# Hamedkiri/heuristique_style_transfer_code

Hardware: NVIDIA B200
Metric: images/sec (higher is better)
Workload: dtype tf32

## Files before the change

heuristique_style_transfer_code_b200/_lib.py:

```python
from __future__ import annotations

import ctypes
import os
from ctypes import c_int, c_longlong, c_void_p, POINTER, c_uint

from .build import LIB_PATH

_LIB = None

GH_DTYPE_F32 = 0
GH_DTYPE_BF16 = 1
GH_ERR_BAD_ARG = -1
GH_ERR_UNSUPPORTED = -2

_P = c_void_p
_SIGNATURES = {
    "gh_version": (c_int, []),
    "gh_sm_count": (c_int, []),
    "gh_set_option": (c_int, [ctypes.c_char_p, c_int]),
    "gh_last_device_error": (c_int, [POINTER(c_uint)]),
    "gh_gram_pool_fwd": (c_int, [_P, c_int, c_longlong, c_longlong, c_longlong, c_int, c_int, c_int, c_int, _P, c_int,
                                  c_int, c_int, c_int, _P]),
    "gh_gram_dense_fwd": (c_int, [_P, c_int, c_longlong, c_longlong, c_longlong, c_int, c_int, c_int, _P, c_int, c_int,
                                   _P]),
    "gh_adaptive_pool_fwd": (c_int, [_P, c_int, c_int, c_int, _P, c_int, c_int, _P]),
    "gh_adaptive_pool_bwd": (c_int, [_P, c_int, c_int, c_int, c_int, c_int, _P, _P]),
    "gh_gram_pool_bwd": (c_int, [_P, c_int, c_longlong, c_longlong, c_longlong, c_int, c_int, c_int, c_int, _P, c_int,
                                  c_int, _P, c_int, c_longlong, c_longlong, c_longlong, c_int, _P]),
    "gh_gram_dense_bwd": (c_int, [_P, c_int, c_longlong, c_longlong, c_longlong, c_int, c_int, c_int, _P, _P, c_int,
                                   c_longlong, c_longlong, c_longlong, c_int, _P]),
    "gh_attn_head_fwd": (c_int, [_P] * 7 + [c_int] * 4 + [_P] * 5 + [_P]),
    "gh_transpose_cast": (c_int, [_P, c_int, _P, c_int, c_int, c_int, c_int, c_longlong, _P]),
    "gh_preprocess_frame": (c_int, [_P, c_longlong, c_int, c_int, c_int, _P, _P, _P, c_int, _P, _P, _P, c_int, _P, _P, _P,
                                     c_int, c_int, _P]),
    "gh_normalize_u8": (c_int, [_P, _P, c_longlong, c_int, c_longlong, _P, _P, _P]),
    "gh_gemm_f32": (c_int, [_P, c_longlong, c_longlong, _P, c_longlong, c_longlong, _P, _P, c_longlong, c_int, c_int,
                             c_int, _P]),
    "gh_maxpool2d_nhwc": (c_int, [_P, c_int, _P] + [c_int] * 7 + [_P]),
    "gh_stem_space_to_depth": (c_int, [_P] + [c_longlong] * 4 + [c_int] * 3 + [_P, c_int, _P]),
    "gh_stem_conv_pool_nhwc": (c_int, [_P] + [c_longlong] * 4 + [c_int] * 3 + [_P] * 4),
    "gh_stem_conv_pool_u8_nhwc": (c_int, [_P] + [c_longlong] * 4 + [c_int] * 3 + [_P] * 6),
    "gh_patch_gram_workspace": (c_longlong, [c_int, c_int, c_int]),
    "gh_patch_gram_fwd": (c_int, [_P, _P, _P, _P, c_int, c_int, c_int, c_int, _P, _P, _P, _P]),
    "gh_patch_attn_fwd": (c_int, [_P] * 11 + [c_int] * 5 + [_P, _P, _P]),
    "gh_attn_head_bwd_workspace": (c_longlong, [c_int, c_int, c_int]),
    "gh_attn_head_bwd": (c_int, [_P] * 10 + [c_int] * 4 + [_P] * 8 + [_P]),
    "gh_gram_mse_blocks": (c_int, [c_longlong]),
    "gh_gram_mse": (c_int, [_P, _P, c_longlong, _P, _P, _P]),
    "gh_split_bf16": (c_int, [_P, _P, c_longlong, c_longlong, _P]),
    "gh_gemm_planes": (c_int, [_P, c_longlong, c_longlong, c_int, _P, c_longlong, c_longlong, c_int, _P, _P, _P,
                                c_longlong, c_longlong, c_int, c_int, c_int, c_int, _P]),
    "gh_tgemm_plan": (c_int, [c_int, c_int, c_int, c_int, c_int, POINTER(c_int), POINTER(c_int), POINTER(c_int)]),
    "gh_gram_bwd_plan": (c_int, [c_int, c_int, c_int, c_int, c_int, POINTER(c_int)]),
    "gh_attn_head_fwd2": (c_int, [_P] * 7 + [c_int] * 4 + [_P] * 6 + [_P]),
    "gh_attn_head_bwd2_workspace": (c_longlong, [c_int, c_int, c_int]),
    "gh_attn_head_bwd2": (c_int, [_P] * 10 + [c_int] * 4 + [_P] * 8 + [_P]),
}
EXPORTED_SYMBOLS = tuple(_SIGNATURES)


class GramHeadError(RuntimeError):
    pass


def library_path() -> str:
    return os.environ.get("GRAMHEAD_LIB", LIB_PATH)


def lib() -> ctypes.CDLL:
    global _LIB
    if _LIB is None:
        path = library_path()
        if not os.path.isfile(path):
            raise GramHeadError(
                f"gramhead: {path} not found. Build it with `python -m heuristique_style_transfer_code_b200.build` "
                "(needs nvcc, targets sm_100a). There is no CPU or PyTorch fallback for the Gram + attention head.")
        handle = ctypes.CDLL(path)
        for name, (res, args) in _SIGNATURES.items():
            fn = getattr(handle, name)
            fn.restype = res
            fn.argtypes = args
        _LIB = handle
        _apply_env_options(handle)
    return _LIB


def _apply_env_options(handle) -> None:
    spec = os.environ.get("GRAMHEAD_OPTIONS", "").strip()
    if not spec:
        return
    for item in spec.split(","):
        name, sep, value = item.strip().partition("=")
        if not sep or not name:
            raise GramHeadError(f"gramhead: GRAMHEAD_OPTIONS: expected name=value, got {item!r}")
# ... 23 lines not shown
```

heuristique_style_transfer_code_b200/build.py:

```python
from __future__ import annotations

import os
import shutil
import subprocess

CSRC = os.path.join(os.path.dirname(os.path.abspath(__file__)), "csrc")
LIB_PATH = os.path.join(CSRC, "libgramhead.so")
SOURCES = ["gramhead.cu", "common.cuh", "gram_fwd.cuh", "pair.cuh", "gram_fwd_pair.cuh", "gram_bwd2.cuh", "gram_bwd_pair.cuh",
           "umma_gemm.cuh", "tgemm_pair.cuh", "launch.cuh", "attn_head.cuh", "attn_head2.cuh", "preprocess.cuh", "transpose.cuh", "patchgan.cuh", "pool.cuh", "stem.cuh", "style_loss.cuh"]
NVCC_FLAGS = ["-gencode", "arch=compute_100a,code=sm_100a", "-O3", "-lineinfo", "-std=c++17",
              "-Xcompiler", "-fPIC", "-shared"]


def _nvcc() -> str:
    for cand in (os.environ.get("NVCC"), shutil.which("nvcc"), "/usr/local/cuda/bin/nvcc"):
        if cand and os.path.isfile(cand):
            return cand
    raise RuntimeError("gramhead: nvcc not found (set NVCC=/path/to/nvcc)")


def is_stale() -> bool:
    if not os.path.isfile(LIB_PATH):
        return True
    built = os.path.getmtime(LIB_PATH)
    deps = [os.path.join(CSRC, s) for s in SOURCES]
    deps.append(os.path.join(os.path.dirname(os.path.dirname(CSRC)), "include", "gramhead.h"))
    return any(os.path.getmtime(d) > built for d in deps if os.path.isfile(d))


def build_library(force: bool = False, verbose: bool = False) -> str:
    if not force and not is_stale():
        return LIB_PATH
    cmd = [_nvcc(), *NVCC_FLAGS, "gramhead.cu", "-o", LIB_PATH + ".tmp"]
    if verbose:
        cmd.insert(1, "-Xptxas=-v")
    res = subprocess.run(cmd, cwd=CSRC, capture_output=True, text=True)
    if res.returncode != 0:
        raise RuntimeError("gramhead: nvcc failed\n" + res.stdout + res.stderr)
    if verbose:
        print(res.stderr)
    os.replace(LIB_PATH + ".tmp", LIB_PATH)
    return LIB_PATH


if __name__ == "__main__":
    print(build_library(force=True, verbose=True))
```

heuristique_style_transfer_code_b200/csrc/gramhead.cu:

```cuda
#include "../../include/gramhead.h"
#include "common.cuh"
#include "gram_fwd.cuh"
#include "gram_fwd_pair.cuh"
#include "gram_bwd2.cuh"
#include "gram_bwd_pair.cuh"
#include "attn_head.cuh"
#include "umma_gemm.cuh"
#include "tgemm_pair.cuh"
#include "attn_head2.cuh"
#include "preprocess.cuh"
#include "transpose.cuh"
#include "patchgan.cuh"
#include "pool.cuh"
#include "stem.cuh"
#include "style_loss.cuh"
#include <string>

namespace gh {

static int sm_count_cached() {
  static int cached[64] = {0};
  int dev = 0;
  if (cudaGetDevice(&dev) != cudaSuccess || dev < 0 || dev >= 64) return 148;
  if (cached[dev] == 0) {
    int n = 0;
    if (cudaDeviceGetAttribute(&n, cudaDevAttrMultiProcessorCount, dev) != cudaSuccess || n <= 0) n = 148;
    cached[dev] = n;
    error_record_host();
  }
  return cached[dev];
}

static int ilog2_exact(int v) {
  if (v <= 0 || (v & (v - 1))) return -1;
  int s = 0;
  while ((1 << s) < v) ++s;
  return s;
}

static int choose_ksplit(long long base_units, int nkb, int ctas, bool balance = false) {
  if (base_units >= ctas) {
    if (!balance) return 1;
    const long long r1 = (base_units + ctas - 1) / ctas * 2, r2 = (2 * base_units + ctas - 1) / ctas;
    return (nkb >= 8 && r2 * 100 <= r1 * 93) ? 2 : 1;
  }
  long long ks = (2LL * ctas + base_units - 1) / base_units;
  const int kmax = nkb / 2 > 1 ? nkb / 2 : 1;
  if (ks > kmax) ks = kmax;
  if (ks > 128) ks = 128;
  return ks < 1 ? 1 : (int)ks;
}

static cudaError_t gemm_auto(const float* A, long long a_sm, long long a_sk, const float* Bm, long long b_sk,
                             long long b_sn, const float* bias, float* D, long long ldd, int M, int N, int K,
                             int accumulate, cudaStream_t st) {
  if (!accumulate && (a_sk == 1 || a_sm == 1) && (b_sk == 1 || b_sn == 1)) {
    const bool a_mn = (a_sk != 1), b_mn = (b_sk != 1);
    cudaError_t e = launch_umma_gemm(A, a_mn, a_mn ? a_sk : a_sm, Bm, b_mn, b_mn ? b_sk : b_sn, bias, D, ldd, M, N, K,
                                     sm_count_cached(), st);
    if (e != cudaErrorNotSupported) return e;
  }
  return launch_sgemm(A, a_sm, a_sk, Bm, b_sk, b_sn, bias, D, ldd, M, N, K, accumulate, st);
}

template <int SRC, int KP>
static cudaError_t launch_gram_fwd_one(const GramFwdParams& p, int grid, cudaStream_t st) {
  cudaError_t e = cudaFuncSetAttribute(gram_fwd_kernel<SRC, KP>, cudaFuncAttributeMaxDynamicSharedMemorySize,
// ... 614 lines not shown
  if (p.OH <= 0 || p.OW <= 0) return GH_ERR_BAD_ARG;
  p.total_vec = (long long)B * p.OH * p.OW * (C / vec);
  const int cv = C / vec;
  if (cv > 256 || B > 65535) return GH_ERR_UNSUPPORTED;
  const int ppc = 256 / cv;
  const dim3 grid((p.OW + ppc - 1) / ppc, (p.OH + kPoolRows - 1) / kPoolRows, B);
  if (grid.y > 65535) return GH_ERR_UNSUPPORTED;
  if (dtype == GH_DTYPE_F32) maxpool2d_nhwc_kernel<float><<<grid, 256, 0, (cudaStream_t)stream>>>(p);
  else maxpool2d_nhwc_kernel<__nv_bfloat16><<<grid, 256, 0, (cudaStream_t)stream>>>(p);
  return (int)cudaGetLastError();
}

int gh_stem_space_to_depth(const float* x, long long img_stride, long long c_stride, long long y_stride,
                           long long x_stride, int B, int H, int W, void* z, int z_dtype, void* stream) {
  if (!x || !z || B <= 0 || H <= 0 || W <= 0) return GH_ERR_BAD_ARG;
  if (z_dtype != GH_DTYPE_F32 && z_dtype != GH_DTYPE_BF16) return GH_ERR_BAD_ARG;
  if ((H & 1) || (W & 1) || (uintptr_t)z % 16 != 0) return GH_ERR_UNSUPPORTED;
  StemS2DParams p{};
  p.x = x; p.z = z; p.s_img = img_stride; p.s_c = c_stride; p.s_y = y_stride; p.s_x = x_stride;
  p.B = B; p.H = H; p.W = W; p.HP = H / 2 + 3; p.WP = W / 2 + 3;
  p.total = (long long)B * p.HP * p.WP;
  const long long want = (p.total + 255) / 256;
  const long long cap = (long long)gh_sm_count() * 32;
  const int grid = (int)(want < cap ? want : cap);
  if (z_dtype == GH_DTYPE_F32) stem_space_to_depth_kernel<float><<<grid, 256, 0, (cudaStream_t)stream>>>(p);
  else stem_space_to_depth_kernel<__nv_bfloat16><<<grid, 256, 0, (cudaStream_t)stream>>>(p);
  return (int)cudaGetLastError();
}

int gh_stem_conv_pool_nhwc(const float* x, long long img_stride, long long c_stride, long long y_stride,
                           long long x_stride, int B, int H, int W, const float* w_packed, const float* bias, float* out,
                           void* stream) {
  if (!x || !w_packed || !bias || !out || B <= 0 || H <= 0 || W <= 0) return GH_ERR_BAD_ARG;
  if ((H & 1) || (W & 1) || (uintptr_t)w_packed % 16 != 0 || (uintptr_t)out % 16 != 0) return GH_ERR_UNSUPPORTED;
  StemConvPoolParams<float> p{};
  p.x = x; p.w = w_packed; p.bias = bias; p.out = out;
  return stem_conv_pool_launch(p, img_stride, c_stride, y_stride, x_stride, B, H, W, stream);
}

int gh_stem_conv_pool_u8_nhwc(const unsigned char* x, long long img_stride, long long c_stride, long long y_stride,
                              long long x_stride, int B, int H, int W, const float* mean3_host, const float* std3_host,
                              const float* w_packed, const float* bias, float* out, void* stream) {
  if (!x || !mean3_host || !std3_host || !w_packed || !bias || !out || B <= 0 || H <= 0 || W <= 0) return GH_ERR_BAD_ARG;
  StemConvPoolParams<uint8_t> p{};
  for (int c = 0; c < 3; ++c) {
    if (!(std3_host[c] != 0.f && std3_host[c] == std3_host[c])) return GH_ERR_BAD_ARG;
    p.mean[c] = mean3_host[c]; p.std[c] = std3_host[c];
  }
  if ((H & 1) || (W & 1) || (uintptr_t)w_packed % 16 != 0 || (uintptr_t)out % 16 != 0) return GH_ERR_UNSUPPORTED;
  p.x = x; p.w = w_packed; p.bias = bias; p.out = out;
  return stem_conv_pool_launch(p, img_stride, c_stride, y_stride, x_stride, B, H, W, stream);
}

int gh_gram_mse_blocks(long long n) {
  if (n <= 0) return 0;
  long long blocks = (n / 4 + kMseThreads - 1) / kMseThreads;
  const long long cap = (long long)sm_count_cached() * 4 < kMseMaxBlocks ? (long long)sm_count_cached() * 4 : kMseMaxBlocks;
  if (blocks > cap) blocks = cap;
  return (int)(blocks < 1 ? 1 : blocks);
}

int gh_gram_mse(const float* G, const float* G_target, long long n, float* dG, float* partial, void* stream) {
  if (!G || !G_target || !dG || !partial || n <= 0) return GH_ERR_BAD_ARG;
  if (n % 4 != 0 || ((uintptr_t)G | (uintptr_t)G_target | (uintptr_t)dG) % 16 != 0) return GH_ERR_UNSUPPORTED;
  gram_mse_kernel<<<gh_gram_mse_blocks(n), kMseThreads, 0, (cudaStream_t)stream>>>(G, G_target, dG, partial, n / 4,
                                                                                   1.0f / (float)n);
  return (int)cudaGetLastError();
}

long long gh_patch_gram_workspace(int L, int B, int D) {
  if (L <= 0 || B <= 0 || D <= 0) return 0;
  return (long long)L * B * D * (kPatchBins + 4);
}

int gh_patch_gram_fwd(const float* const* maps, const int* H, const int* W, const long long* strides, int L, int B,
                      int D, int ln_input, float* gram, float* gram_norm, float* workspace, void* stream) {
  if (!maps || !H || !W || !strides || !gram || !gram_norm || !workspace || L <= 0 || B <= 0 || D <= 0)
    return GH_ERR_BAD_ARG;
  if ((uintptr_t)workspace % 8 != 0) return GH_ERR_BAD_ARG;
  if (L > kPatchMaxLayers || D > kPatchMaxD || B > 0x7fffffff / 2) return GH_ERR_UNSUPPORTED;
  PatchGramParams p{};
  for (int l = 0; l < L; ++l) {
    if (!maps[l] || H[l] <= 0 || W[l] <= 0) return GH_ERR_BAD_ARG;
    p.layer[l].x = maps[l];
    p.layer[l].H = H[l];
    p.layer[l].W = W[l];
    p.layer[l].s_img = strides[4 * l + 0];
    p.layer[l].s_c = strides[4 * l + 1];
    p.layer[l].s_y = strides[4 * l + 2];
    p.layer[l].s_x = strides[4 * l + 3];
  }
  p.L = L; p.B = B; p.D = D; p.ln_input = ln_input ? 1 : 0;
  p.gram = gram; p.gram_norm = gram_norm;
  const long long planes = (long long)L * B * D;
  double* stats = reinterpret_cast<double*>(workspace);
  float* pooled = workspace + planes * 4;
  const long long gx = (long long)B * ((D + 7) / 8);
  if (gx > 0x7fffffffLL) return GH_ERR_UNSUPPORTED;
  patch_pool_kernel<<<dim3((unsigned)gx, L), kPatchThreads, (kPatchThreads / 32) * kPatchSmallPlane * sizeof(float),
                      (cudaStream_t)stream>>>(p, pooled, stats);
  cudaError_t e = cudaGetLastError();
  if (e != cudaSuccess) return (int)e;
  const size_t smem = (size_t)D * kPatchBins * 4 + 32 * sizeof(double);
  patch_gram_kernel<<<dim3(B, L), kPatchThreads, smem, (cudaStream_t)stream>>>(p, pooled, stats);
  return (int)cudaGetLastError();
}
// ... 240 lines not shown
```

heuristique_style_transfer_code_b200/frozen_encoder.py:

```python
from __future__ import annotations

import os
from typing import List, Optional, Tuple

import torch
import torch.nn as nn
import torch.nn.functional as F

from . import ops

STEM_SPACE_TO_DEPTH = os.environ.get("GRAMHEAD_STEM_S2D", "1") != "0"


def _stem_space_to_depth_weight(weight: torch.Tensor) -> torch.Tensor:
    o = weight.shape[0]
    w8 = weight.new_zeros((o, 3, 8, 8))
    w8[:, :, 1:, 1:] = weight
    w12 = w8.view(o, 3, 4, 2, 4, 2).permute(0, 1, 3, 5, 2, 4).reshape(o, 12, 4, 4)
    w16 = weight.new_zeros((o, 16, 4, 4))
    w16[:, :12] = w12
    return w16.contiguous(memory_format=torch.channels_last)


def _tf32_round(x: torch.Tensor) -> torch.Tensor:
    bits = (x.contiguous().view(torch.int32).to(torch.int64) & 0xFFFFFFFF) + 0x1000
    bits = bits & 0xFFFFE000
    return torch.where(bits >= 2 ** 31, bits - 2 ** 32, bits).to(torch.int32).view(torch.float32)


def pack_stem_weight(w16: torch.Tensor) -> torch.Tensor:
    w = _tf32_round(w16.float().contiguous())
    return w.view(64, 2, 2, 4, 4, 4).permute(4, 5, 1, 2, 0, 3).contiguous().view(-1)


def _fold(conv: nn.Conv2d, bn: nn.BatchNorm2d, dtype: torch.dtype, channels_last: bool):
    var, mean = bn.running_var.detach().float(), bn.running_mean.detach().float()
    gamma = bn.weight.detach().float() if bn.weight is not None else torch.ones_like(var)
    beta = bn.bias.detach().float() if bn.bias is not None else torch.zeros_like(var)
    scale = gamma * torch.rsqrt(var + bn.eps)
    weight = conv.weight.detach().float() * scale.view(-1, 1, 1, 1)
    bias = beta - mean * scale
    if conv.bias is not None:
        bias = bias + conv.bias.detach().float() * scale
    weight = weight.to(dtype).contiguous(memory_format=torch.channels_last if channels_last else torch.contiguous_format)
    return weight, bias.to(dtype).contiguous(), conv.stride, conv.padding, conv.dilation, conv.groups


def _foldable(conv, bn) -> bool:
    return (isinstance(conv, nn.Conv2d) and type(bn) is nn.BatchNorm2d and bn.track_running_stats
            and bn.running_mean is not None and bn.running_var is not None and conv.padding_mode == "zeros"
            and not isinstance(conv.padding, str))


def _is_bottleneck(block) -> bool:
    names = ("conv1", "bn1", "conv2", "bn2", "conv3", "bn3", "relu", "downsample")
    if type(block).__name__ != "Bottleneck" or not all(hasattr(block, n) for n in names):
        return False
    if not isinstance(block.relu, nn.ReLU):
        return False
    ok = _foldable(block.conv1, block.bn1) and _foldable(block.conv2, block.bn2) and _foldable(block.conv3, block.bn3)
    if block.downsample is not None:
        ds = block.downsample
        ok = ok and isinstance(ds, nn.Sequential) and len(ds) == 2 and _foldable(ds[0], ds[1])
    return ok


def encoder_signature(encoder: nn.Module) -> Optional[Tuple]:
    try:
        return tuple((t.data_ptr(), t._version) for t in list(encoder.parameters()) + list(encoder.buffers()))
    except RuntimeError:
        return None


class FoldedEncoder:

    def __init__(self, stem, pool, stages, signature, dtype, channels_last):
        self.stem, self.pool, self.stages = stem, pool, stages
        self.stem_s2d = None
        self.stem_packed = None
        self._stem_fused = True
        self.signature, self.dtype, self.channels_last = signature, dtype, channels_last

    @staticmethod
    def supported(encoder: nn.Sequential) -> bool:
        if len(encoder) < 4:
            return False
        if not (_foldable(encoder[0], encoder[1]) and isinstance(encoder[2], nn.ReLU) and isinstance(encoder[3], nn.MaxPool2d)):
            return False
        for stage in list(encoder)[4:]:
            if not isinstance(stage, nn.Sequential) or not all(_is_bottleneck(b) for b in stage):
                return False
        return True

    @classmethod
    def build(cls, encoder: nn.Sequential, dtype: torch.dtype, channels_last: bool) -> Optional["FoldedEncoder"]:
        if not cls.supported(encoder):
            return None
        with torch.no_grad():
            stem = _fold(encoder[0], encoder[1], dtype, channels_last)
            conv1 = encoder[0]
            stem_s2d = None
            if (STEM_SPACE_TO_DEPTH and channels_last and conv1.in_channels == 3 and conv1.kernel_size == (7, 7)
                    and conv1.stride == (2, 2) and conv1.padding == (3, 3) and conv1.dilation == (1, 1) and conv1.groups == 1):
                stem_s2d = (_stem_space_to_depth_weight(stem[0].float()).to(dtype), stem[1], (1, 1), (0, 0), (1, 1), 1)
            stages: List[list] = []
            for stage in list(encoder)[4:]:
                blocks = []
                for b in stage:
                    c3 = _fold(b.conv3, b.bn3, dtype, channels_last)
                    down = None
                    if b.downsample is not None:
                        dw, db, *geom = _fold(b.downsample[0], b.downsample[1], torch.float32, channels_last)
                        bias3 = (c3[1].float() + db).to(dtype)
                        c3 = (c3[0], bias3) + tuple(c3[2:])
                        down = (dw.to(dtype).contiguous(memory_format=torch.channels_last if channels_last
                                                        else torch.contiguous_format), None) + tuple(geom)
                    blocks.append((_fold(b.conv1, b.bn1, dtype, channels_last), _fold(b.conv2, b.bn2, dtype, channels_last),
                                   c3, down))
                stages.append(blocks)
        plan = cls(stem, encoder[3], stages, encoder_signature(encoder), dtype, channels_last)
        plan.stem_s2d = stem_s2d
        pool = encoder[3]
        if (stem_s2d is not None and dtype == torch.float32 and conv1.out_channels == 64
                and pool.kernel_size in (3, (3, 3)) and pool.stride in (2, (2, 2)) and pool.padding in (1, (1, 1))
                and pool.dilation in (1, (1, 1)) and not pool.ceil_mode and not pool.return_indices):
            plan.stem_packed = pack_stem_weight(stem_s2d[0])
        return plan

    @staticmethod
    def _conv_relu(x, p):
        w, b, stride, padding, dilation, groups = p
        return torch.cudnn_convolution_relu(x, w, b, stride, padding, dilation, groups)

    def _pool(self, x):
        p = self.pool
        k, s, pad = p.kernel_size, p.stride, p.padding
        plain = (isinstance(k, int) and isinstance(s, int) and isinstance(pad, int) and p.dilation == 1
                 and not p.ceil_mode and not p.return_indices)
        vec = 4 if x.dtype == torch.float32 else 8
        if plain and self.channels_last and x.shape[1] % vec == 0 and x.is_contiguous(memory_format=torch.channels_last):
            return ops.maxpool2d_nhwc(x, k, s, pad)
        return p(x)

    def _fused_stem_applies(self, x: torch.Tensor) -> bool:
        return (self.stem_packed is not None and self._stem_fused and torch.backends.cudnn.allow_tf32
                and x.dim() == 4 and x.shape[1] == 3 and x.shape[2] % 2 == 0 and x.shape[3] % 2 == 0)

    def stem_forward(self, x: torch.Tensor, normalize=None) -> torch.Tensor:
        if normalize is not None and x.dtype == torch.uint8:
            if self._fused_stem_applies(x):
                return ops.stem_conv_pool_u8(x, *normalize, self.stem_packed, self.stem_s2d[1])
            x = ops.normalize_u8(x, *normalize)
        if x.dtype == torch.float32 and self._fused_stem_applies(x):
            return ops.stem_conv_pool(x, self.stem_packed, self.stem_s2d[1])
        if (self.stem_s2d is not None and x.dtype == torch.float32 and x.shape[1] == 3 and x.shape[2] % 2 == 0
                and x.shape[3] % 2 == 0):
            x = self._conv_relu(ops.stem_space_to_depth(x, self.dtype), self.stem_s2d)
        else:
            x = x.to(self.dtype)
            if self.channels_last:
                x = x.contiguous(memory_format=torch.channels_last)
            x = self._conv_relu(x, self.stem)
        return self._pool(x)

    def __call__(self, x: torch.Tensor, normalize=None):
        x = self.stem_forward(x, normalize)
        outs = []
        for blocks in self.stages:
            for c1, c2, c3, down in blocks:
                identity = x
                y = self._conv_relu(x, c1)
                y = self._conv_relu(y, c2)
                if down is not None:
                    identity = F.conv2d(x, down[0], down[1], down[2], down[3], down[4], down[5])
                w, b, stride, padding, dilation, groups = c3
                x = torch.cudnn_convolution_add_relu(y, w, identity, 1.0, b, stride, padding, dilation, groups)
            outs.append(x)
        return x, outs
```

heuristique_style_transfer_code_b200/ops.py:

```python
from __future__ import annotations

import ctypes
from typing import List, Optional, Sequence, Tuple

import torch

from . import _lib
from ._lib import GH_DTYPE_BF16, GH_DTYPE_F32, GramHeadError, check

KSPLIT = 0
MAX_CTAS = 0

LAUNCHES = 0
PROFILE = None


class _Timed:
    def __init__(self, name, kernels, device, **work):
        self.name, self.kernels, self.device, self.work = name, kernels, device, work

    def __enter__(self):
        global LAUNCHES
        LAUNCHES += self.kernels
        if PROFILE is not None:
# ... 201 lines not shown
    with torch.cuda.device(a.device), _Timed(f"gemm_f32[M={m},N={n},K={k}]", 1, a.device, **work):
        rc = _lib.lib().gh_gemm_f32(a.data_ptr(), a.stride(0), a.stride(1), b.data_ptr(), b.stride(0), b.stride(1),
                                    0 if bias is None else bias.data_ptr(), out.data_ptr(), n, m, n, k, _stream_ptr(a))
    check(rc, "gh_gemm_f32")
    return out


def maxpool2d_nhwc(x: torch.Tensor, kernel: int, stride: int, padding: int) -> torch.Tensor:
    _require_cuda(x, "x")
    if x.dim() != 4 or not x.is_contiguous(memory_format=torch.channels_last):
        raise GramHeadError("gramhead: maxpool2d_nhwc takes a channels_last (B, C, H, W) tensor")
    b, c, h, w = x.shape
    oh, ow = (h + 2 * padding - kernel) // stride + 1, (w + 2 * padding - kernel) // stride + 1
    out = torch.empty((b, c, oh, ow), device=x.device, dtype=x.dtype, memory_format=torch.channels_last)
    work = dict(bytes=(x.numel() + out.numel()) * x.element_size(), flops=0, kind="maxpool")
    with torch.cuda.device(x.device), _Timed(f"maxpool2d_nhwc[C={c},HW={h}x{w},{x.dtype}]", 1, x.device, **work):
        rc = _lib.lib().gh_maxpool2d_nhwc(x.data_ptr(), _dtype_code(x), out.data_ptr(), b, h, w, c, kernel, stride, padding,
                                          _stream_ptr(x))
    check(rc, "gh_maxpool2d_nhwc")
    return out


def stem_space_to_depth(x: torch.Tensor, dtype: torch.dtype) -> torch.Tensor:
    _require_cuda(x, "x")
    if x.dim() != 4 or x.shape[1] != 3 or x.dtype != torch.float32 or x.shape[2] % 2 or x.shape[3] % 2:
        raise GramHeadError("gramhead: stem_space_to_depth takes fp32 (B, 3, H, W) images with even H and W")
    b, _, h, w = x.shape
    z = torch.empty((b, 16, h // 2 + 3, w // 2 + 3), device=x.device, dtype=dtype, memory_format=torch.channels_last)
    work = dict(bytes=x.numel() * 4 + z.numel() * z.element_size(), flops=0, kind="stem_s2d")
    with torch.cuda.device(x.device), _Timed(f"stem_space_to_depth[HW={h}x{w},{dtype}]", 1, x.device, **work):
        rc = _lib.lib().gh_stem_space_to_depth(x.data_ptr(), x.stride(0), x.stride(1), x.stride(2), x.stride(3), b, h, w,
                                               z.data_ptr(), _dtype_code(z), _stream_ptr(x))
    check(rc, "gh_stem_space_to_depth")
    return z


def stem_conv_pool(x: torch.Tensor, packed_weight: torch.Tensor, bias: torch.Tensor) -> torch.Tensor:
    _require_cuda(x, "x")
    if x.dim() != 4 or x.shape[1] != 3 or x.dtype != torch.float32 or x.shape[2] % 2 or x.shape[3] % 2:
        raise GramHeadError("gramhead: stem_conv_pool takes fp32 (B, 3, H, W) images with even H and W")
    if (packed_weight.dtype != torch.float32 or packed_weight.numel() != 16384 or not packed_weight.is_contiguous()
            or bias.dtype != torch.float32 or bias.numel() != 64 or not bias.is_contiguous()
            or packed_weight.device != x.device or bias.device != x.device):
        raise GramHeadError("gramhead: stem_conv_pool takes the packed fp32 stem weights (16384) and bias (64) on x's device")
    b, _, h, w = x.shape
    oh, ow = h // 2, w // 2
    ph, pw = (oh - 1) // 2 + 1, (ow - 1) // 2 + 1
    out = torch.empty((b, 64, ph, pw), device=x.device, dtype=torch.float32, memory_format=torch.channels_last)
    work = dict(bytes=(x.numel() + out.numel()) * 4, flops=2 * b * oh * ow * 64 * 147, kind="stem_conv_pool")
    with torch.cuda.device(x.device), _Timed(f"stem_conv_pool[HW={h}x{w}]", 1, x.device, **work):
        rc = _lib.lib().gh_stem_conv_pool_nhwc(x.data_ptr(), x.stride(0), x.stride(1), x.stride(2), x.stride(3), b, h, w,
                                               packed_weight.data_ptr(), bias.data_ptr(), out.data_ptr(), _stream_ptr(x))
    check(rc, "gh_stem_conv_pool_nhwc")
    return out


def stem_conv_pool_u8(x: torch.Tensor, mean, std, packed_weight: torch.Tensor, bias: torch.Tensor) -> torch.Tensor:
    _require_cuda(x, "x")
    if x.dim() != 4 or x.shape[1] != 3 or x.dtype != torch.uint8 or x.shape[2] % 2 or x.shape[3] % 2:
        raise GramHeadError("gramhead: stem_conv_pool_u8 takes uint8 (B, 3, H, W) images with even H and W")
    if (packed_weight.dtype != torch.float32 or packed_weight.numel() != 16384 or not packed_weight.is_contiguous()
            or bias.dtype != torch.float32 or bias.numel() != 64 or not bias.is_contiguous()
            or packed_weight.device != x.device or bias.device != x.device):
        raise GramHeadError("gramhead: stem_conv_pool_u8 takes the packed fp32 stem weights (16384) and bias (64) on x's device")
    mean, std = [float(v) for v in mean], [float(v) for v in std]
    if len(mean) != 3 or len(std) != 3:
        raise GramHeadError("gramhead: stem_conv_pool_u8: 3 channels need 3 means and stds")
    b, _, h, w = x.shape
    oh, ow = h // 2, w // 2
    ph, pw = (oh - 1) // 2 + 1, (ow - 1) // 2 + 1
    out = torch.empty((b, 64, ph, pw), device=x.device, dtype=torch.float32, memory_format=torch.channels_last)
    fl = ctypes.c_float * 3
    work = dict(bytes=x.numel() + out.numel() * 4, flops=2 * b * oh * ow * 64 * 147, kind="stem_conv_pool")
    with torch.cuda.device(x.device), _Timed(f"stem_conv_pool_u8[HW={h}x{w}]", 1, x.device, **work):
        rc = _lib.lib().gh_stem_conv_pool_u8_nhwc(x.data_ptr(), x.stride(0), x.stride(1), x.stride(2), x.stride(3), b, h,
                                                  w, fl(*mean), fl(*std), packed_weight.data_ptr(), bias.data_ptr(),
                                                  out.data_ptr(), _stream_ptr(x))
    check(rc, "gh_stem_conv_pool_u8_nhwc")
    return out


def normalize_u8_host(t: torch.Tensor, mean, std) -> torch.Tensor:
    shape = (1, -1, 1, 1)
    out = t.to(torch.float32).div_(255)
    return out.sub_(torch.tensor(mean, dtype=torch.float32).view(shape)).div_(torch.tensor(std, dtype=torch.float32).view(shape))


def normalize_u8(x: torch.Tensor, mean, std, out: Optional[torch.Tensor] = None) -> torch.Tensor:
    _require_cuda(x, "x")
    if x.dim() != 4 or x.dtype != torch.uint8 or not 1 <= x.shape[1] <= 4:
        raise GramHeadError("gramhead: normalize_u8 takes a (B, C <= 4, H, W) uint8 batch")
    mean, std = [float(v) for v in mean], [float(v) for v in std]
    b, c, h, w = x.shape
    if len(mean) != c or len(std) != c:
        raise GramHeadError(f"gramhead: normalize_u8: {c} channels need {c} means and stds")
    x = x.contiguous()
    if out is None:
        out = torch.empty((b, c, h, w), device=x.device, dtype=torch.float32)
    else:
        if (out.dtype != torch.float32 or out.device != x.device or out.dim() != 4 or out.shape[0] < b
                or out.shape[1:] != x.shape[1:] or not out.is_contiguous()):
            raise GramHeadError("gramhead: normalize_u8: `out` must be a dense fp32 (>= B, C, H, W) tensor on x's device")
        out = out[:b]
    if b == 0:
        return out
    fl = ctypes.c_float * c
# ... 349 lines not shown
```

include/gramhead.h:

```cpp
#ifndef GRAMHEAD_H_
#define GRAMHEAD_H_

#ifdef __cplusplus
extern "C" {
#endif

#define GH_ERR_BAD_ARG (-1)
#define GH_ERR_UNSUPPORTED (-2)

#define GH_DTYPE_F32 0
#define GH_DTYPE_BF16 1

int gh_version(void);

int gh_sm_count(void);

int gh_set_option(const char* name, int value);

int gh_last_device_error(unsigned int* out4);

int gh_gram_pool_fwd(const void* F, int f_dtype, long long img_stride, long long row_stride, long long x_stride, int B,
                     int C, int HW, int g, float* desc, int l, int L, int ksplit, int max_ctas, void* stream);

int gh_gram_dense_fwd(const void* F, int f_dtype, long long img_stride, long long row_stride, long long x_stride, int B,
                      int C, int HW, float* G, int ksplit, int max_ctas, void* stream);

int gh_adaptive_pool_fwd(const float* G, int B, int C, int g, float* desc, int l, int L, void* stream);
int gh_adaptive_pool_bwd(const float* d_desc, int l, int L, int B, int C, int g, float* dG, void* stream);

int gh_gram_pool_bwd(const void* F, int f_dtype, long long img_stride, long long row_stride, long long x_stride, int B,
                     int C, int HW, int g, const float* d_desc, int l, int L, void* dF, int df_dtype,
                     long long df_img_stride, long long df_row_stride, long long df_x_stride, int max_ctas, void* stream);

int gh_gram_dense_bwd(const void* F, int f_dtype, long long img_stride, long long row_stride, long long x_stride, int B,
                      int C, int HW, const float* dG, void* dF, int df_dtype, long long df_img_stride,
                      long long df_row_stride, long long df_x_stride, int max_ctas, void* stream);

int gh_attn_head_fwd(const float* desc, const float* W_in, const float* b_in, const float* W_out, const float* b_out,
                     const float* W_c, const float* b_c, int B, int L, int E, int nc, float* qkv, float* probs,
                     float* obar, float* emb, float* logits, void* stream);

int gh_transpose_cast(const void* in, int in_dtype, void* out, int out_dtype, int B, int R, int S, long long out_pitch,
                      void* stream);

int gh_preprocess_frame(const unsigned char* frame, long long pitch_bytes, int H, int W, int bgr, const int* hx_min,
                        const int* hx_size, const int* hk, int hkmax, const int* vy_min, const int* vy_size, const int* vk,
                        int vkmax, const float* mean3_host, const float* std3_host, float* out, int OH, int OW,
                        void* stream);

int gh_normalize_u8(const unsigned char* src, float* dst, long long images, int channels, long long hw,
                    const float* mean_host, const float* std_host, void* stream);

int gh_gemm_f32(const float* A, long long a_sm, long long a_sk, const float* B, long long b_sk, long long b_sn,
                const float* bias, float* D, long long ldd, int M, int N, int K, void* stream);

int gh_maxpool2d_nhwc(const void* in, int dtype, void* out, int B, int H, int W, int C, int k, int stride, int pad,
                      void* stream);

int gh_stem_space_to_depth(const float* x, long long img_stride, long long c_stride, long long y_stride,
                           long long x_stride, int B, int H, int W, void* z, int z_dtype, void* stream);

int gh_stem_conv_pool_nhwc(const float* x, long long img_stride, long long c_stride, long long y_stride,
                           long long x_stride, int B, int H, int W, const float* w_packed, const float* bias, float* out,
                           void* stream);

int gh_stem_conv_pool_u8_nhwc(const unsigned char* x, long long img_stride, long long c_stride, long long y_stride,
                              long long x_stride, int B, int H, int W, const float* mean3_host, const float* std3_host,
                              const float* w_packed, const float* bias, float* out, void* stream);

long long gh_patch_gram_workspace(int L, int B, int D);
int gh_patch_gram_fwd(const float* const* maps, const int* H, const int* W, const long long* strides, int L, int B,
                      int D, int ln_input, float* gram, float* gram_norm, float* workspace, void* stream);

int gh_patch_attn_fwd(const float* feat, const float* W_in1, const float* b_in1, const float* W_out1,
                      const float* b_out1, const float* W_in2, const float* b_in2, const float* W_out2,
                      const float* b_out2, const float* W_c, const float* b_c, int L, int B, int E, int heads, int nc,
                      float* emb, float* logits, void* stream);

long long gh_attn_head_bwd_workspace(int B, int L, int E);

int gh_attn_head_bwd(const float* desc, const float* W_in, const float* W_out, const float* W_c, const float* qkv,
                     const float* probs, const float* obar, const float* emb, const float* d_logits,
                     const float* d_emb_ext, int B, int L, int E, int nc, float* d_desc, float* dW_in, float* db_in,
                     float* dW_out, float* db_out, float* dW_c, float* db_c, float* workspace, void* stream);

int gh_gram_mse_blocks(long long n);
int gh_gram_mse(const float* G, const float* G_target, long long n, float* dG, float* partial, void* stream);

int gh_split_bf16(const float* src, void* planes, long long n, long long plane_stride, void* stream);

int gh_gemm_planes(const void* A_planes, long long lda, long long a_plane_stride, int a_mn, const void* B_planes,
                   long long ldb, long long b_plane_stride, int b_mn, const float* bias, float* D, void* D_planes,
                   long long ldd, long long d_plane_stride, int M, int N, int K, int max_split, void* stream);

int gh_tgemm_plan(int M, int N, int K, int max_split, int npairs, int* tn, int* ksplit, int* units);

int gh_gram_bwd_plan(int C, int HW, int g, int f_dtype, int channels_last, int* out);

int gh_attn_head_fwd2(const float* desc, const void* w_in_planes, const float* b_in, const void* w_out_planes,
                      const float* b_out, const float* W_c, const float* b_c, int B, int L, int E, int nc, void* x_planes,
                      float* qkv, float* probs, void* obar_planes, float* emb, float* logits, void* stream);

long long gh_attn_head_bwd2_workspace(int B, int L, int E);

int gh_attn_head_bwd2(const void* x_planes, const void* w_in_planes, const void* w_out_planes, const float* W_c,
                      const float* qkv, const float* probs, const void* obar_planes, const float* emb,
                      const float* d_logits, const float* d_emb_ext, int B, int L, int E, int nc, float* d_desc,
                      float* dW_in, float* db_in, float* dW_out, float* db_out, float* dW_c, float* db_c, void* workspace,
                      void* stream);

#ifdef __cplusplus
}
#endif
#endif
```

Baseline: 46110.

## Fuse ResNet downsample shortcut and conv3 into one tcgen05 GEMM kernel

Adds a warp-specialized tcgen05 TF32 GEMM kernel that computes the first bottleneck block's 1x1 conv3 and 1x1 downsample shortcut as one K=128 GEMM over the concatenated inputs, then applies bias, the residual sum and ReLU from TMEM in a single pass. This replaces a separate downsample conv, an intermediate identity tensor and a cuDNN conv-add-relu call, cutting memory traffic and launches for that block. It applies only to fp32 channels_last blocks with 64->256 1x1 convs. Producer warps load and TF32-round the activations into shared memory, accumulators are double-buffered in TMEM, and the weights stay resident in shared memory. Summing the two bias vectors is assumed to happen when the packed bias is built.

```diff
diff --git a/heuristique_style_transfer_code_b200/_lib.py b/heuristique_style_transfer_code_b200/_lib.py
--- a/heuristique_style_transfer_code_b200/_lib.py
+++ b/heuristique_style_transfer_code_b200/_lib.py
@@ -40,6 +40,7 @@
     "gh_stem_space_to_depth": (c_int, [_P] + [c_longlong] * 4 + [c_int] * 3 + [_P, c_int, _P]),
     "gh_stem_conv_pool_nhwc": (c_int, [_P] + [c_longlong] * 4 + [c_int] * 3 + [_P] * 4),
     "gh_stem_conv_pool_u8_nhwc": (c_int, [_P] + [c_longlong] * 4 + [c_int] * 3 + [_P] * 6),
+    "gh_conv3_shortcut_relu_nhwc": (c_int, [_P, _P, c_longlong, _P, _P, _P, _P]),
     "gh_patch_gram_workspace": (c_longlong, [c_int, c_int, c_int]),
     "gh_patch_gram_fwd": (c_int, [_P, _P, _P, _P, c_int, c_int, c_int, c_int, _P, _P, _P, _P]),
     "gh_patch_attn_fwd": (c_int, [_P] * 11 + [c_int] * 5 + [_P, _P, _P]),
diff --git a/heuristique_style_transfer_code_b200/build.py b/heuristique_style_transfer_code_b200/build.py
--- a/heuristique_style_transfer_code_b200/build.py
+++ b/heuristique_style_transfer_code_b200/build.py
@@ -7,7 +7,8 @@
 CSRC = os.path.join(os.path.dirname(os.path.abspath(__file__)), "csrc")
 LIB_PATH = os.path.join(CSRC, "libgramhead.so")
 SOURCES = ["gramhead.cu", "common.cuh", "gram_fwd.cuh", "pair.cuh", "gram_fwd_pair.cuh", "gram_bwd2.cuh", "gram_bwd_pair.cuh",
-           "umma_gemm.cuh", "tgemm_pair.cuh", "launch.cuh", "attn_head.cuh", "attn_head2.cuh", "preprocess.cuh", "transpose.cuh", "patchgan.cuh", "pool.cuh", "stem.cuh", "style_loss.cuh"]
+           "umma_gemm.cuh", "tgemm_pair.cuh", "launch.cuh", "attn_head.cuh", "attn_head2.cuh", "preprocess.cuh", "transpose.cuh", "patchgan.cuh", "pool.cuh", "stem.cuh", "conv3_shortcut.cuh",
+           "style_loss.cuh"]
 NVCC_FLAGS = ["-gencode", "arch=compute_100a,code=sm_100a", "-O3", "-lineinfo", "-std=c++17",
               "-Xcompiler", "-fPIC", "-shared"]
 
diff --git a/heuristique_style_transfer_code_b200/csrc/conv3_shortcut.cuh b/heuristique_style_transfer_code_b200/csrc/conv3_shortcut.cuh
--- /dev/null
+++ b/heuristique_style_transfer_code_b200/csrc/conv3_shortcut.cuh
@@ -0,0 +1,167 @@
+#pragma once
+#include "common.cuh"
+
+namespace gh {
+
+constexpr int kCsProducerWarps = 4;
+constexpr int kCsEpiWarp0 = kCsProducerWarps;
+constexpr int kCsEpiWarps = 8;
+constexpr int kCsMmaWarp = kCsEpiWarp0 + kCsEpiWarps;
+constexpr int kCsThreads = (kCsMmaWarp + 1) * 32;
+constexpr int kCsSlots = 3;
+constexpr uint32_t kCsWBytes = 32 * 256 * 16;
+constexpr uint32_t kCsSlotBytes = 16 * 128 * 16;
+constexpr uint32_t kCsAOff = kCsWBytes;
+constexpr uint32_t kCsBiasOff = kCsAOff + kCsSlots * kCsSlotBytes;
+constexpr uint32_t kCsBarOff = kCsBiasOff + 256 * 4;
+constexpr uint32_t kCsBarBytes = 8 * (2 * kCsSlots + 2 * 2) + 16;
+constexpr uint32_t kCsSmemBytes = kCsBarOff + kCsBarBytes + 1024;
+static_assert(kCsSmemBytes <= 232448, "conv3_shortcut: shared memory budget");
+
+struct Conv3ShortcutParams {
+  const float* y;
+  const float* x;
+  const float* w;
+  const float* bias;
+  float* out;
+  long long M;
+  int tiles;
+};
+
+__device__ __forceinline__ float cs_max_nan(float a, float b) {
+  float r;
+  asm("max.NaN.f32 %0, %1, %2;" : "=f"(r) : "f"(a), "f"(b));
+  return r;
+}
+
+__global__ void __launch_bounds__(kCsThreads, 1) conv3_shortcut_kernel(const Conv3ShortcutParams p) {
+  extern __shared__ uint8_t smem_raw[];
+  const uint32_t raw = smem_u32(smem_raw);
+  const uint32_t base = (raw + 1023u) & ~1023u;
+  uint8_t* gbase = smem_raw + (base - raw);
+  const uint32_t w_smem = base, a_smem = base + kCsAOff;
+  const float* bias_s = reinterpret_cast<const float*>(gbase + kCsBiasOff);
+  const uint32_t bar_full = base + kCsBarOff, bar_empty = bar_full + 8 * kCsSlots;
+  const uint32_t bar_afull = bar_empty + 8 * kCsSlots, bar_aempty = bar_afull + 16;
+  const uint32_t tmem_slot = bar_aempty + 16;
+  volatile uint32_t* tmem_slot_ptr = reinterpret_cast<volatile uint32_t*>(gbase + (tmem_slot - base));
+  const int warp = threadIdx.x >> 5, lane = threadIdx.x & 31;
+
+  {
+    const float4* wg = reinterpret_cast<const float4*>(p.w);
+    float4* ws = reinterpret_cast<float4*>(gbase);
+    for (int i = threadIdx.x; i < (int)(kCsWBytes / 16); i += kCsThreads) ws[i] = __ldg(wg + i);
+    if (threadIdx.x < 256) reinterpret_cast<float*>(gbase + kCsBiasOff)[threadIdx.x] = __ldg(p.bias + threadIdx.x);
+    fence_proxy_async_smem();
+  }
+  if (threadIdx.x == 0) {
+    for (int s = 0; s < kCsSlots; ++s) {
+      mbar_init(bar_full + 8 * s, kCsProducerWarps);
+      mbar_init(bar_empty + 8 * s, 1);
+    }
+    for (int s = 0; s < 2; ++s) {
+      mbar_init(bar_afull + 8 * s, 1);
+      mbar_init(bar_aempty + 8 * s, kCsEpiWarps);
+    }
+    mbar_fence_init();
+  }
+  if (warp == kCsMmaWarp) tmem_alloc(tmem_slot, 512);
+  tc_fence_before_sync();
+  __syncthreads();
+  tc_fence_after_sync();
+  const uint32_t tmem_base = *tmem_slot_ptr;
+
+  if (warp < kCsProducerWarps) {
+    const int r_lo = lane & 7, q = 4 * warp + (lane >> 3);
+    uint32_t g = 0;
+    for (int t = blockIdx.x; t < p.tiles; t += gridDim.x) {
+      const long long m0 = (long long)t * 128;
+#pragma unroll 1
+      for (int src = 0; src < 2; ++src, ++g) {
+        const float* s = (src == 0 ? p.y : p.x) + q * 4;
+        float4 v[16];
+#pragma unroll
+        for (int r_hi = 0; r_hi < 16; ++r_hi) {
+          const long long m = m0 + r_hi * 8 + r_lo;
+          v[r_hi] = m < p.M ? __ldg(reinterpret_cast<const float4*>(s + m * 64)) : make_float4(0.f, 0.f, 0.f, 0.f);
+        }
+        const uint32_t slot = g % kCsSlots;
+        mbar_wait(bar_empty + 8 * slot, ((g / kCsSlots) & 1u) ^ 1u, 700u + slot);
+        const uint32_t dst = a_smem + slot * kCsSlotBytes + (uint32_t)q * 2048u + (uint32_t)r_lo * 16u;
+#pragma unroll
+        for (int r_hi = 0; r_hi < 16; ++r_hi)
+          sts_u4(dst + (uint32_t)r_hi * 128u, tf32_rna(v[r_hi].x), tf32_rna(v[r_hi].y), tf32_rna(v[r_hi].z),
+                 tf32_rna(v[r_hi].w));
+        fence_proxy_async_smem();
+        __syncwarp();
+        if (lane == 0) mbar_arrive(bar_full + 8 * slot);
+      }
+    }
+  } else if (warp == kCsMmaWarp) {
+    constexpr uint32_t idesc = make_idesc_tf32(128, 256);
+    const uint64_t adesc = make_smem_desc_noswz(a_smem, 2048, 128);
+    const uint64_t bdesc = make_smem_desc_noswz(w_smem, 4096, 128);
+    uint32_t g = 0, i = 0;
+    for (int t = blockIdx.x; t < p.tiles; t += gridDim.x, ++i, g += 2) {
+      const uint32_t acc = i & 1u;
+      mbar_wait(bar_aempty + 8 * acc, ((i >> 1) & 1u) ^ 1u, 800u + acc);
+      const uint32_t sy = g % kCsSlots, sx = (g + 1) % kCsSlots;
+      mbar_wait(bar_full + 8 * sy, (g / kCsSlots) & 1u, 810u + sy);
+      mbar_wait(bar_full + 8 * sx, ((g + 1) / kCsSlots) & 1u, 810u + sx);
+      tc_fence_after_sync();
+      if (elect_one()) {
+        const uint32_t d = tmem_base + acc * 256u;
+#pragma unroll
+        for (int c = 0; c < 8; ++c)
+          umma_tf32(d, adesc + ((sy * kCsSlotBytes + c * 4096u) >> 4), bdesc + ((c * 8192u) >> 4), idesc, c != 0);
+#pragma unroll
+        for (int c = 0; c < 8; ++c)
+          umma_tf32(d, adesc + ((sx * kCsSlotBytes + c * 4096u) >> 4), bdesc + ((65536u + c * 8192u) >> 4), idesc, 1u);
+        umma_commit(bar_afull + 8 * acc);
+        umma_commit(bar_empty + 8 * sy);
+        umma_commit(bar_empty + 8 * sx);
+      }
+      __syncwarp();
+    }
+  } else {
+    const int quad = warp & 3, half = (warp - kCsEpiWarp0) >> 2;
+    const uint32_t tlane = tmem_base + ((uint32_t)(32 * quad) << 16) + 128u * (uint32_t)half;
+    const float* bias_h = bias_s + 128 * half;
+    uint32_t i = 0;
+    for (int t = blockIdx.x; t < p.tiles; t += gridDim.x, ++i) {
+      const uint32_t acc = i & 1u;
+      mbar_wait(bar_afull + 8 * acc, (i >> 1) & 1u, 900u + acc);
+      tc_fence_after_sync();
+      const long long m = (long long)t * 128 + 32 * quad + lane;
+      float4* o = reinterpret_cast<float4*>(p.out + m * 256 + 128 * half);
+#pragma unroll 1
+      for (int cc = 0; cc < 4; ++cc) {
+        uint32_t r[32];
+        tmem_ld32_nowait(tlane + acc * 256u + 32u * (uint32_t)cc, r);
+        tmem_ld_wait();
+        if (m < p.M) {
+#pragma unroll
+          for (int e = 0; e < 32; e += 4) {
+            const float* b = bias_h + 32 * cc + e;
+            o[(32 * cc + e) / 4] = make_float4(cs_max_nan(__uint_as_float(r[e]) + b[0], 0.f),
+                                               cs_max_nan(__uint_as_float(r[e + 1]) + b[1], 0.f),
+                                               cs_max_nan(__uint_as_float(r[e + 2]) + b[2], 0.f),
+                                               cs_max_nan(__uint_as_float(r[e + 3]) + b[3], 0.f));
+          }
+        }
+      }
+      tc_fence_before_sync();
+      __syncwarp();
+      if (lane == 0) mbar_arrive(bar_aempty + 8 * acc);
+    }
+  }
+
+  tc_fence_before_sync();
+  __syncthreads();
+  if (warp == kCsMmaWarp) {
+    tc_fence_after_sync();
+    tmem_dealloc(tmem_base, 512);
+  }
+}
+
+}
diff --git a/heuristique_style_transfer_code_b200/csrc/gramhead.cu b/heuristique_style_transfer_code_b200/csrc/gramhead.cu
--- a/heuristique_style_transfer_code_b200/csrc/gramhead.cu
+++ b/heuristique_style_transfer_code_b200/csrc/gramhead.cu
@@ -13,6 +13,7 @@
 #include "patchgan.cuh"
 #include "pool.cuh"
 #include "stem.cuh"
+#include "conv3_shortcut.cuh"
 #include "style_loss.cuh"
 #include <string>
 
@@ -733,6 +734,24 @@
   return stem_conv_pool_launch(p, img_stride, c_stride, y_stride, x_stride, B, H, W, stream);
 }
 
+int gh_conv3_shortcut_relu_nhwc(const float* y, const float* x, long long M, const float* w_packed, const float* bias,
+                                float* out, void* stream) {
+  if (!y || !x || !w_packed || !bias || !out || M <= 0) return GH_ERR_BAD_ARG;
+  if ((uintptr_t)y % 16 != 0 || (uintptr_t)x % 16 != 0 || (uintptr_t)w_packed % 16 != 0 || (uintptr_t)out % 16 != 0)
+    return GH_ERR_BAD_ARG;
+  const long long tiles = (M + 127) / 128;
+  if (tiles >= (1ll << 30)) return GH_ERR_BAD_ARG;
+  Conv3ShortcutParams p{};
+  p.y = y; p.x = x; p.w = w_packed; p.bias = bias; p.out = out; p.M = M; p.tiles = (int)tiles;
+  const int sms = sm_count_cached();
+  const int grid = p.tiles < sms ? p.tiles : sms;
+  cudaError_t e = cudaFuncSetAttribute(conv3_shortcut_kernel, cudaFuncAttributeMaxDynamicSharedMemorySize,
+                                       (int)kCsSmemBytes);
+  if (e != cudaSuccess) return (int)e;
+  conv3_shortcut_kernel<<<grid, kCsThreads, kCsSmemBytes, (cudaStream_t)stream>>>(p);
+  return (int)cudaGetLastError();
+}
+
 int gh_gram_mse_blocks(long long n) {
   if (n <= 0) return 0;
   long long blocks = (n / 4 + kMseThreads - 1) / kMseThreads;
diff --git a/heuristique_style_transfer_code_b200/frozen_encoder.py b/heuristique_style_transfer_code_b200/frozen_encoder.py
--- a/heuristique_style_transfer_code_b200/frozen_encoder.py
+++ b/heuristique_style_transfer_code_b200/frozen_encoder.py
@@ -31,6 +31,17 @@
 def pack_stem_weight(w16: torch.Tensor) -> torch.Tensor:
     w = _tf32_round(w16.float().contiguous())
     return w.view(64, 2, 2, 4, 4, 4).permute(4, 5, 1, 2, 0, 3).contiguous().view(-1)
+
+
+def pack_conv3_shortcut_weight(w3: torch.Tensor, wd: torch.Tensor) -> torch.Tensor:
+    w = _tf32_round(torch.cat([w3.float().reshape(256, 64), wd.float().reshape(256, 64)], dim=1).contiguous())
+    return w.view(256, 32, 4).permute(1, 0, 2).contiguous().view(-1)
+
+
+def _is_1x1(p, cin: int, cout: int) -> bool:
+    w, _, stride, padding, dilation, groups = p
+    return (tuple(w.shape) == (cout, cin, 1, 1) and tuple(stride) == (1, 1) and tuple(padding) == (0, 0)
+            and tuple(dilation) == (1, 1) and groups == 1)
 
 
 def _fold(conv: nn.Conv2d, bn: nn.BatchNorm2d, dtype: torch.dtype, channels_last: bool):
@@ -79,6 +90,8 @@
         self.stem_s2d = None
         self.stem_packed = None
         self._stem_fused = True
+        self.tail_packed = {}
+        self._tail_fused = True
         self.signature, self.dtype, self.channels_last = signature, dtype, channels_last
 
     @staticmethod
@@ -125,6 +138,11 @@
                 and pool.kernel_size in (3, (3, 3)) and pool.stride in (2, (2, 2)) and pool.padding in (1, (1, 1))
                 and pool.dilation in (1, (1, 1)) and not pool.ceil_mode and not pool.return_indices):
             plan.stem_packed = pack_stem_weight(stem_s2d[0])
+        if dtype == torch.float32 and channels_last:
+            for si, blocks in enumerate(stages):
+                for bi, (_, _, c3, down) in enumerate(blocks):
+                    if down is not None and _is_1x1(c3, 64, 256) and _is_1x1(down, 64, 256):
+                        plan.tail_packed[(si, bi)] = pack_conv3_shortcut_weight(c3[0], down[0])
         return plan
 
     @staticmethod
@@ -163,17 +181,26 @@
             x = self._conv_relu(x, self.stem)
         return self._pool(x)
 
+    def block_forward(self, x: torch.Tensor, block, tail_packed: Optional[torch.Tensor] = None) -> torch.Tensor:
+        c1, c2, c3, down = block
+        identity = x
+        y = self._conv_relu(x, c1)
+        y = self._conv_relu(y, c2)
+        if (tail_packed is not None and self._tail_fused and torch.backends.cudnn.allow_tf32
+                and x.dtype == torch.float32 and y.dtype == torch.float32 and x.dim() == 4 and x.shape == y.shape
+                and x.is_contiguous(memory_format=torch.channels_last)
+                and y.is_contiguous(memory_format=torch.channels_last)):
+            return ops.conv3_shortcut_relu(y, x, tail_packed, c3[1])
+        if down is not None:
+            identity = F.conv2d(x, down[0], down[1], down[2], down[3], down[4], down[5])
+        w, b, stride, padding, dilation, groups = c3
+        return torch.cudnn_convolution_add_relu(y, w, identity, 1.0, b, stride, padding, dilation, groups)
+
     def __call__(self, x: torch.Tensor, normalize=None):
         x = self.stem_forward(x, normalize)
         outs = []
-        for blocks in self.stages:
-            for c1, c2, c3, down in blocks:
-                identity = x
-                y = self._conv_relu(x, c1)
-                y = self._conv_relu(y, c2)
-                if down is not None:
-                    identity = F.conv2d(x, down[0], down[1], down[2], down[3], down[4], down[5])
-                w, b, stride, padding, dilation, groups = c3
-                x = torch.cudnn_convolution_add_relu(y, w, identity, 1.0, b, stride, padding, dilation, groups)
+        for si, blocks in enumerate(self.stages):
+            for bi, block in enumerate(blocks):
+                x = self.block_forward(x, block, self.tail_packed.get((si, bi)))
             outs.append(x)
         return x, outs
diff --git a/heuristique_style_transfer_code_b200/ops.py b/heuristique_style_transfer_code_b200/ops.py
--- a/heuristique_style_transfer_code_b200/ops.py
+++ b/heuristique_style_transfer_code_b200/ops.py
@@ -277,6 +277,27 @@
         rc = _lib.lib().gh_stem_conv_pool_nhwc(x.data_ptr(), x.stride(0), x.stride(1), x.stride(2), x.stride(3), b, h, w,
                                                packed_weight.data_ptr(), bias.data_ptr(), out.data_ptr(), _stream_ptr(x))
     check(rc, "gh_stem_conv_pool_nhwc")
+    return out
+
+
+def conv3_shortcut_relu(y: torch.Tensor, x: torch.Tensor, packed_weight: torch.Tensor, bias: torch.Tensor) -> torch.Tensor:
+    _require_cuda(y, "y")
+    if (y.dim() != 4 or y.shape[1] != 64 or y.dtype != torch.float32 or x.shape != y.shape or x.dtype != torch.float32
+            or x.device != y.device or not y.is_contiguous(memory_format=torch.channels_last)
+            or not x.is_contiguous(memory_format=torch.channels_last)):
+        raise GramHeadError("gramhead: conv3_shortcut_relu takes two channels_last fp32 (B, 64, H, W) tensors of one shape")
+    if (packed_weight.dtype != torch.float32 or packed_weight.numel() != 32768 or not packed_weight.is_contiguous()
+            or bias.dtype != torch.float32 or bias.numel() != 256 or not bias.is_contiguous()
+            or packed_weight.device != y.device or bias.device != y.device):
+        raise GramHeadError("gramhead: conv3_shortcut_relu takes the packed fp32 weights (32768) and bias (256) on y's device")
+    b, _, h, w = y.shape
+    m = b * h * w
+    out = torch.empty((b, 256, h, w), device=y.device, dtype=torch.float32, memory_format=torch.channels_last)
+    work = dict(bytes=(y.numel() + x.numel() + out.numel()) * 4, flops=2 * m * 128 * 256, kind="conv3_shortcut")
+    with torch.cuda.device(y.device), _Timed(f"conv3_shortcut_relu[HW={h}x{w}]", 1, y.device, **work):
+        rc = _lib.lib().gh_conv3_shortcut_relu_nhwc(y.data_ptr(), x.data_ptr(), m, packed_weight.data_ptr(),
+                                                    bias.data_ptr(), out.data_ptr(), _stream_ptr(y))
+    check(rc, "gh_conv3_shortcut_relu_nhwc")
     return out
 
 
diff --git a/include/gramhead.h b/include/gramhead.h
--- a/include/gramhead.h
+++ b/include/gramhead.h
@@ -68,6 +68,9 @@
                               long long x_stride, int B, int H, int W, const float* mean3_host, const float* std3_host,
                               const float* w_packed, const float* bias, float* out, void* stream);
 
+int gh_conv3_shortcut_relu_nhwc(const float* y, const float* x, long long M, const float* w_packed, const float* bias,
+                                float* out, void* stream);
+
 long long gh_patch_gram_workspace(int L, int B, int D);
 int gh_patch_gram_fwd(const float* const* maps, const int* H, const int* W, const long long* strides, int L, int B,
                       int D, int ln_input, float* gram, float* gram_norm, float* workspace, void* stream);
```

Result: no change. 46230, median of 6 (+0.3%).
